# FlyCole/Dream2Real

Hardware: AMD Instinct MI355X
Metric: candidate renders scored/sec (640x360) (higher is better)
Workload: dtype bf16 + fp16 NeRF MLP operands (fp32 accumulate; the library's default: the reference's tiny-cuda-nn operand type, same MFMA rate; --opt mlp_f16=0 = bf16 operands)

## Files before the change

### dream2real_amd/_lib.py

```python
from __future__ import annotations

import ctypes as C
import os

import numpy as np

_HERE = os.path.dirname(os.path.abspath(__file__))
LIB_PATH = os.path.join(_HERE, "libd2r.so")
ABI_VERSION = 10

EXPORTS = [
    "d2r_abi_version", "d2r_ctx_create", "d2r_ctx_destroy", "d2r_ctx_set_stream", "d2r_ctx_synchronize",
    "d2r_last_error", "d2r_nerf_create", "d2r_nerf_destroy", "d2r_render", "d2r_nerf_eval_points",
    "d2r_set_background", "d2r_render_composite", "d2r_clip_create", "d2r_clip_destroy",
    "d2r_clip_score_frames", "d2r_clip_preprocess", "d2r_clip_embed_pixels", "d2r_render_score",
    "d2r_get_render_stats", "d2r_collect_render_stats", "d2r_ctx_set_option", "d2r_get_timing", "d2r_text_create",
    "d2r_text_destroy", "d2r_text_encode", "d2r_comm_get_unique_id", "d2r_comm_init", "d2r_comm_destroy",
    "d2r_allgather_scores", "d2r_phys_create", "d2r_phys_destroy", "d2r_phys_check", "d2r_nerf_load_ingp", "d2r_lens_undistort_view",
    "d2r_rectify_background_depth", "d2r_ingp_inspect", "d2r_render_score_host", "d2r_png_write", "d2r_png_write_batch",
    "d2r_png_read_batch", "d2r_png_size", "d2r_savetxt", "d2r_ingp_validate", "d2r_debug_gemm_fp8", "d2r_ctx_get_option", "d2r_png_write_batch_bg",
    "d2r_pcd_create", "d2r_pcd_destroy", "d2r_pcd_render", "d2r_pcd_render_score_host",
    "d2r_tsdf_create", "d2r_tsdf_destroy", "d2r_tsdf_integrate", "d2r_tsdf_read_voxels", "d2r_tsdf_extract", "d2r_obj_write",
    "d2r_tsdf_grid", "d2r_tsdf_touch_bits", "d2r_tsdf_solid_points",
    "d2r_sdfphys_create", "d2r_sdfphys_destroy", "d2r_sdfphys_check", "d2r_sdfphys_get_timing",
    "d2r_png_write_channels", "d2r_png_info", "d2r_png_read_grey", "d2r_png_read_rgb",
    "d2r_scene_bound_masks", "d2r_masks_prune", "d2r_masks_components", "d2r_masks_lut", "d2r_masks_get_timing",
    "d2r_pcd_build", "d2r_pcd_size", "d2r_pcd_read", "d2r_pcd_build_get_timing",
    "d2r_masks_census",
]


class D2RError(RuntimeError):
    pass


class NerfDesc(C.Structure):
    _fields_ = [("n_levels", C.c_uint32), ("n_features", C.c_uint32), ("level_scale", C.c_void_p),
                ("level_res", C.c_void_p), ("level_size", C.c_void_p), ("level_offset", C.c_void_p),
                ("n_entries", C.c_uint32), ("grid_fp16", C.c_void_p), ("dw1_fp16", C.c_void_p),
                ("dw2_fp16", C.c_void_p), ("cw1_fp16", C.c_void_p), ("cw2_fp16", C.c_void_p),
                ("cw3_fp16", C.c_void_p), ("occupancy_bits", C.c_void_p), ("aabb_scale", C.c_uint32),
                ("render_aabb", C.c_float * 6)]

# ... 308 lines not shown

def pcd_build_timing(ctx):
    ms = np.zeros(2, np.float64)
    check(load().d2r_pcd_build_get_timing(_h(ctx), ptr(ms)), _h(ctx))
    return tuple(float(x) for x in ms)


def ingp_validate(data: bytes) -> IngpInfo:
    info = IngpInfo()
    lib = load()
    lib.d2r_ingp_validate.argtypes = [C.c_char_p, C.c_size_t, C.c_void_p]
    check(lib.d2r_ingp_validate(data, len(data), C.byref(info)))
    return info


def check(rc: int, ctx=None):
    if rc != 0:
        msg = load().d2r_last_error(ctx)
        raise D2RError(f"libd2r error {rc}: {msg.decode() if msg else '?'}")


def ptr(a) -> C.c_void_p:
    if a is None:
        return C.c_void_p(0)
    assert a.flags["C_CONTIGUOUS"]
    return C.c_void_p(a.ctypes.data)


def view_c(v) -> ViewC:
    return ViewC(v.width, v.height, (C.c_float * 2)(*v.focal), (C.c_float * 2)(*v.center), v.scale,
# ... 3 lines not shown
```

### dream2real_amd/csrc/api.hip

```cpp
#include <math.h>
#include <string.h>

#include <algorithm>
#include <chrono>

#include "d2r_internal.h"
#include "pngio.h"

struct d2r_clip;
int d2r_launch_preprocess(d2r_ctx *, d2r_clip *, const uint8_t *frames_dev, uint32_t n, uint32_t w, uint32_t h,
                          int rot90, uint16_t *patches_dev, float *pixel_values_dev, const void *rects_dev = nullptr,
                          const uint16_t *bg_patches_dev = nullptr, bool touched_only = false);
bool d2r_clip_l0_supported(const d2r_ctx *, const d2r_clip *);
int d2r_clip_forward(d2r_ctx *, const d2r_clip *, const uint16_t *patches_dev, uint32_t n, const float *text_dev,
                     uint32_t C, float logit_scale, float *logits_dev, float *embeds_dev, const ClipL0Reuse *reuse = nullptr);
int d2r_clip_layer0_background(d2r_ctx *, const d2r_clip *, const uint16_t *bg_patches_dev, ClipL0Reuse *out);
int d2r_launch_patchify(d2r_ctx *, const d2r_clip *, const float *pv_dev, uint32_t n, uint16_t *patches_dev);
size_t d2r_clip_patch_bytes(const d2r_clip *, uint32_t n);
int d2r_launch_eval_points(d2r_ctx *, const d2r_nerf *, const float *xyz, const float *dirs, uint32_t n, float *out);
uint32_t d2r_clip_image_size(const d2r_clip *);
uint32_t d2r_clip_proj_dim(const d2r_clip *);
uint32_t d2r_clip_max_images(const d2r_clip *);
uint32_t d2r_clip_tokens(const d2r_clip *);

uint32_t d2r_pass_size(const d2r_ctx *ctx, const d2r_clip *clip, size_t px)
{
    uint64_t per = (uint64_t)std::max<int64_t>(1, ctx->chunk);
// ... 140 lines not shown
    {"ray_sort_log2", &d2r_ctx::ray_sort_log2, Option::RANGE, 1, 4},
    {"march_threads", &d2r_ctx::march_threads, Option::RANGE, 0, D2R_MARCH_THREADS, 0, opt_march_threads},
    {"march_threads_auto_mib", &d2r_ctx::march_threads_auto_mib, Option::RANGE, 0, 1 << 20},
    {"march_blocks", &d2r_ctx::march_blocks, Option::RANGE, 0, 65535},
    {"gemm_cfg", &d2r_ctx::gemm_cfg, Option::FREE, 0, 0, OPT_DEV},
    {"gemm_group", &d2r_ctx::gemm_group, Option::RANGE, 0, 65535, OPT_DEV},
    {"gemm_stagger", &d2r_ctx::gemm_stagger, Option::FLAG, 0, 0, OPT_DEV},
    {"gbrick_slots", &d2r_ctx::gbrick_slots, Option::RANGE, 0, 8},
    {"brick_slots_total", &d2r_ctx::brick_slots_total, Option::RANGE, 0, 8},
    {"lds_slots_max", &d2r_ctx::lds_slots_max, Option::RANGE, 0, 5},
    {"gbrick_max_mib", &d2r_ctx::gbrick_max_mib, Option::RANGE, 0, 512},
    {"mlp_f16", &d2r_ctx::mlp_f16, Option::FLAG},
    {"render_arith", &d2r_ctx::render_arith, Option::RANGE, 0, 2},
    {"bricks", &d2r_ctx::use_bricks, Option::FLAG},
    {"raygen_rect", &d2r_ctx::raygen_rect, Option::FLAG},
    {"timing", &d2r_ctx::timing, Option::RANGE, 0, 2, 0, opt_timing},
    {"march_lds_slots", &d2r_ctx::last_march_nb, Option::FREE, 0, 0, OPT_READ_ONLY},
    {"march_hbm_brick_slots", &d2r_ctx::last_march_ngb, Option::FREE, 0, 0, OPT_READ_ONLY},
    {"march_hbm_brick_bytes", &d2r_ctx::last_march_gbrick_bytes, Option::FREE, 0, 0, OPT_READ_ONLY},
    {"march_threads_used", &d2r_ctx::last_march_threads, Option::FREE, 0, 0, OPT_READ_ONLY},
};

static const Option *find_option(const char *key)
{
    for (const Option &o : g_options)
        if (!strcmp(key, o.key)) return (o.flags & OPT_DEV) && !kDevBuild ? nullptr : &o;
    return nullptr;
}

size_t d2r_ctx::timing_begin(int kind)
// ... 749 lines not shown
    ClipL0Reuse l0{};
    const bool use_l0 = reuse_bg && ctx->l0_reuse && d2r_clip_l0_supported(ctx, clip);
    if (use_l0) {
        if (ctx->bg_l0_for != (const void *)clip) {
            rc = d2r_clip_layer0_background(ctx, clip, (const uint16_t *)ctx->bg_patches.p, &ctx->bg_l0_desc);
            if (rc == D2R_OK) ctx->bg_l0_for = (const void *)clip;
            else if (rc != D2R_ERR_UNSUPPORTED) return rc;
        }
        if (ctx->bg_l0_for == (const void *)clip) {
            l0 = ctx->bg_l0_desc;
            l0.w = V.W;
            l0.h = V.H;
            l0.rects = ctx->rects.p;
        }
    }
    ctx->stats = d2r_render_stats{};
    hipStream_t main = ctx->stream, rs = two ? ctx->render_stream : main, xs = ctx->copy_stream;
    if (rs != main) {
        D2R_HIP(ctx, hipEventRecord(ctx->ev_fork, main));
        D2R_HIP(ctx, hipStreamWaitEvent(rs, ctx->ev_fork, 0));
    }
    uint32_t prev_c0 = 0, prev_nc = 0;
    int prev_b = -1;
    for (uint32_t c0 = 0, ci = 0; c0 < K; c0 += per, ci++) {
        const uint32_t nc = std::min(per, K - c0);
        const int b = (int)(ci & 1u), pb = two ? b : 0, fbuf = (to_host && nchunks > 1) ? b : 0;
        uint8_t *frames_dev = (uint8_t *)(fbuf ? ctx->frames2.p : ctx->frames.p);
        uint16_t *patches = (uint16_t *)(pb ? ctx->patches2.p : ctx->clipws[6].p);
        void *rects = reuse_bg ? (void *)((uint8_t *)ctx->rects.p + (size_t)pb * cap * 16) : nullptr;
        if (to_host && ci >= 2) ctx->pool->wait(b);
        {
            StreamSwap sw(ctx, rs);
            if (to_host && ci >= 2) D2R_HIP(ctx, hipStreamWaitEvent(rs, ctx->ev_copy[b], 0));
            if (two && ci >= 2) D2R_HIP(ctx, hipStreamWaitEvent(rs, ctx->ev_clip[pb], 0));
            if ((rc = d2r_launch_cameras_virtual(ctx, V, obj_pose_now, cam_pose, poses_dev + (size_t)c0 * 16, nc, (float *)ctx->cams.p)))
                return rc;
            if ((rc = d2r_launch_render(ctx, fg, V, (const float *)ctx->cams.p, nc, true, nullptr, nullptr, frames_dev, rects)))
                return rc;
            D2R_HIP(ctx, hipMemcpyAsync((uint8_t *)ctx->counters.p + 64 + 32 * (size_t)ci, ctx->counters.p, 32,
                                        hipMemcpyDeviceToDevice, rs));
            if (ctx->debug_fail_chunk >= 0 && (int64_t)ci == ctx->debug_fail_chunk) {
                ctx->debug_fail_chunk = -1;
                return d2r_fail(ctx, D2R_ERR_DEVICE, "injected fault in chunk " + std::to_string(ci) + " (option debug_fail_chunk)");
            }
            size_t tp = ctx->timing_begin(D2R_T_PREP);
            if ((rc = d2r_launch_preprocess(ctx, (d2r_clip *)clip, frames_dev, nc, V.W, V.H, 1, patches, nullptr, rects,
                                            reuse_bg ? (const uint16_t *)ctx->bg_patches.p : nullptr, l0.rects != nullptr)))
                return rc;
            ctx->timing_end(tp);
            if (to_host) {
                D2R_HIP(ctx, hipEventRecord(ctx->ev_march[b], rs));
                D2R_HIP(ctx, hipStreamWaitEvent(xs, ctx->ev_march[b], 0));
// ... 127 lines not shown
    ctx->stats.samples = 0;
    ctx->stats.wave_iters = 0;
    ctx->stats.l0_touched = 0;
    for (uint32_t i = 0; i < nchunks; i++) {
        if (ctx->stats.l0_tokens) ctx->stats.l0_touched += c[i * 8 + 6];
        uint64_t s, it;
        memcpy(&s, &c[i * 8 + 2], 8);
        memcpy(&it, &c[i * 8 + 4], 8);
        ctx->stats.rays_alive += c[i * 8];
        ctx->stats.samples += s;
        ctx->stats.wave_iters += it;
    }
    return D2R_OK;
}

}
```

### dream2real_amd/csrc/clip.hip

```cpp
#include "d2r_internal.h"

#include <type_traits>

#include <math.h>
#include <stdio.h>
#include <stdlib.h>

#include <algorithm>
#include <deque>
#include <mutex>

typedef __bf16 bf16x8 __attribute__((ext_vector_type(8)));
typedef float f32x16 __attribute__((ext_vector_type(16)));
typedef float f32x4 __attribute__((ext_vector_type(4)));

struct ClipWeights {
    const uint16_t *w_patch;
    const float *cls, *pos;
    const float *pre_w, *pre_b;
    struct Layer {
        const float *ln1_w, *ln1_b, *ln2_w, *ln2_b;
        const uint16_t *w_qkv, *w_o, *w_fc1, *w_fc2;
        const float *b_qkv, *b_o, *b_fc1, *b_fc2;
        const uint16_t *wf_qkv = nullptr, *wf_fc1 = nullptr;
// ... 9 lines not shown
    const int *kk_h;
    const int *bounds_v;
    const int *kk_v;
    int ks_h, ks_v;
    int need_h, need_v;
    int iw, ih;
    int rw, rh;
    int left, top;
    int max_rows;
};

struct PrepCache {
    uint32_t w, h;
    int rot90;
    ResampleTables R;
};

struct d2r_clip {
    d2r_ctx *ctx;
    d2r_clip_desc desc;
    uint32_t T, Kp, Kp_pad;
    std::vector<void *> allocs;
    ClipWeights w;
    std::vector<ClipWeights::Layer> layers;
    std::deque<PrepCache> prep;
    std::mutex prep_mu;
    struct F8Layer { const uint8_t *w_qkv, *w_o, *w_fc1, *w_fc2; float s_qkv, s_o, s_fc1, s_fc2; };
    std::vector<F8Layer> f8;
    std::mutex f8_mu;
};
// ... 2416 lines not shown
        for (int x = 0; x < xmax; x++) {
            k[x] = bicubic_filter((x + xmin - center + 0.5) * ss);
            ww += k[x];
        }
        for (int x = 0; x < ksize; x++) {
            double v = x < xmax ? (ww != 0.0 ? k[x] / ww : k[x]) : 0.0;
            kk[(size_t)xx * ksize + x] = v < 0 ? (int)(-0.5 + v * (1 << PRECISION_BITS))
                                               : (int)(0.5 + v * (1 << PRECISION_BITS));
        }
        bounds[xx * 2] = xmin;
        bounds[xx * 2 + 1] = xmax;
    }
    return ksize;
}

static int prep_tables(d2r_ctx *ctx, d2r_clip *clip, uint32_t w, uint32_t h, int rot90, const PrepCache **out)
{
    std::lock_guard<std::mutex> lock(clip->prep_mu);
    for (const PrepCache &pc : clip->prep)
        if (pc.w == w && pc.h == h && pc.rot90 == rot90) {
            *out = &pc;
            return D2R_OK;
        }
    const uint32_t S = clip->desc.image_size, P = clip->desc.patch_size;
    ResampleTables R{};
    R.iw = rot90 ? (int)h : (int)w;
    R.ih = rot90 ? (int)w : (int)h;
    int short_e = R.iw < R.ih ? R.iw : R.ih, long_e = R.iw < R.ih ? R.ih : R.iw;
    int new_long = (int)((double)S * long_e / short_e);
    R.rw = R.iw <= R.ih ? (int)S : new_long;
    R.rh = R.iw <= R.ih ? new_long : (int)S;
    R.need_h = R.rw != R.iw;
    R.need_v = R.rh != R.ih;
    R.left = (R.rw - (int)S) / 2;
    R.top = (R.rh - (int)S) / 2;
    std::vector<int> bh, kh, bv, kv;
    R.ks_h = resample_coeffs(R.iw, R.rw, bh, kh);
    R.ks_v = resample_coeffs(R.ih, R.rh, bv, kv);
    const uint32_t band = P;
    int max_rows = (int)band;
    if (R.need_v) {
        max_rows = 0;
        for (uint32_t r0 = 0; r0 < S; r0 += band) {
            uint32_t last = std::min(r0 + band, S) - 1;
            int y0 = bv[2 * (R.top + r0)], y1 = bv[2 * (R.top + last)] + bv[2 * (R.top + last) + 1];
            max_rows = std::max(max_rows, y1 - y0);
        }
    }
    R.max_rows = max_rows;
    std::vector<int> all;
    size_t o_bh = 0, o_kh = o_bh + bh.size(), o_bv = o_kh + kh.size(), o_kv = o_bv + bv.size();
    all.insert(all.end(), bh.begin(), bh.end());
    all.insert(all.end(), kh.begin(), kh.end());
    all.insert(all.end(), bv.begin(), bv.end());
    all.insert(all.end(), kv.begin(), kv.end());
    int *dev = nullptr;
    if (hipMalloc(&dev, all.size() * sizeof(int)) != hipSuccess) return d2r_fail(ctx, D2R_ERR_MEMORY, "hipMalloc failed");
    clip->allocs.push_back(dev);
    D2R_HIP(ctx, hipMemcpy(dev, all.data(), all.size() * sizeof(int), hipMemcpyHostToDevice));
    R.bounds_h = dev + o_bh;
    R.kk_h = dev + o_kh;
    R.bounds_v = dev + o_bv;
    R.kk_v = dev + o_kv;
    clip->prep.push_back(PrepCache{w, h, rot90, R});
    *out = &clip->prep.back();
    return D2R_OK;
}

int d2r_launch_preprocess(d2r_ctx *ctx, d2r_clip *clip, const uint8_t *frames_dev, uint32_t n, uint32_t w,
                          uint32_t h, int rot90, uint16_t *patches_dev, float *pixel_values_dev, const void *rects_dev,
                          const uint16_t *bg_patches_dev, bool touched_only)
{
    const uint32_t S = clip->desc.image_size, P = clip->desc.patch_size;
    const PrepCache *pc = nullptr;
    int rc = prep_tables(ctx, clip, w, h, rot90, &pc);
    if (rc) return rc;
    const ResampleTables &R = pc->R;
    const uint32_t band = P;
    size_t lds = (size_t)R.max_rows * S * 3;
    if (lds > 150 * 1024) return d2r_fail(ctx, D2R_ERR_UNSUPPORTED, "preprocess band does not fit in LDS");
// ... 823 lines not shown
```

### dream2real_amd/csrc/d2r_internal.h

```cpp
#pragma once
#include <hip/hip_runtime.h>
#include <stdint.h>

#include <functional>
#include <memory>
#include <mutex>
#include <string>
#include <utility>
#include <vector>

#include "../../include/d2r.h"
#include "d2r_shared.h"

class D2rJobPool;
struct D2rPngBase;

#define D2R_MAX_LEVELS 16
#define D2R_MAX_DEVICES 64
#define D2R_GRID 128
#define D2R_DT 0.0016914558f
#define D2R_INV_DT (1.0f / D2R_DT)
#define D2R_CONE 0.00390625f
#define D2R_T_LINEAR (D2R_DT * 256.0f)
#define D2R_N_WFRAG 24
// ... 13 lines not shown
    uint32_t hashed[2];
    uint32_t mask8;
    uint32_t off;
    uint32_t bnx[2], bnxy[2];
    int32_t bbase[2];
};

struct NerfParams {
    const uint32_t *grid;
    uint32_t grid_bytes;
    uint32_t n_levels;
    int32_t n_dense;
    SlotMeta slot[D2R_MAX_LEVELS / 2];
    uint32_t refill_min;
    uint32_t compact;
    uint32_t sort_log2;
    uint32_t n_brick_slots;
    uint32_t brick_words;
    const uint32_t *brick_tab;
    uint32_t n_gbrick_slots;
    uint32_t gbrick_bytes;
    const uint32_t *gbrick_tab;
    const uint64_t *bricks;
    uint32_t aabb_scale;
    uint32_t n_casc;
    float side, inv_side;
    const uint4 *wfrag;
    const uint4 *wfrag16;
    float bbox_lo[3], bbox_hi[3];
    float raabb_lo[3], raabb_hi[3], rn_lo[3], rn_hi[3];
// ... 82 lines not shown
    int64_t last_march_threads = 0, last_march_gbrick_bytes = 0;
    int64_t last_march_nb = 0, last_march_ngb = 0;
    int64_t refill_min = 64;
    int64_t march_compact = 1;
    int64_t ln_fold = 4;
    int64_t gemm_stagger = 0;
    int64_t gemm_group = 65535;
    int64_t gemm_nsplit = 0;
    int64_t attn_rem = 1;
    int64_t cls_last = 1;
    int64_t gemm_cfg = 0;
    int64_t mlp_f16 = 1;
    int64_t render_arith = 0;
    int64_t use_bricks = 1;
    int64_t raygen_rect = 1;
    int64_t gbrick_slots = 8;
    int64_t brick_slots_total = 7;
    int64_t lds_slots_max = 5;
    int64_t gbrick_max_mib = 512;
    int64_t timing = 0;
    std::vector<hipEvent_t> ev_pool;
    size_t ev_used = 0;
    std::vector<std::pair<int, std::pair<size_t, size_t>>> ev_pairs;
    size_t timing_begin(int kind);
    void timing_end(size_t pair);
};
enum { D2R_T_MARCH = 0, D2R_T_RAYGEN = 1, D2R_T_CLIP = 2, D2R_T_PREP = 3, D2R_T_SORT = 4,
       D2R_T_VIT_QKV = 5, D2R_T_VIT_ATTN = 6, D2R_T_VIT_OUT = 7, D2R_T_VIT_FC1 = 8, D2R_T_VIT_FC2 = 9, D2R_T_KINDS = 10 };

struct d2r_nerf {
// ... 34 lines not shown
#define D2R_HIP(ctx, expr)                                                              \
    do {                                                                                \
        hipError_t e_ = (expr);                                                         \
        if (e_ != hipSuccess)                                                           \
            return d2r_fail(ctx, D2R_ERR_DEVICE,                                        \
                            std::string(#expr) + ": " + hipGetErrorString(e_));         \
    } while (0)

int d2r_launch_cameras_direct(d2r_ctx *, const ViewParams &, const float *cams_nerf_dev, uint32_t n,
                              float *cams_out);
int d2r_launch_cameras_virtual(d2r_ctx *, const ViewParams &, const float *obj_now16,
                               const float *cam16, const float *obj_poses_dev, uint32_t n,
                               float *cams_out);
int d2r_launch_render(d2r_ctx *, const d2r_nerf *, const ViewParams &, const float *cams_dev,
                      uint32_t n, bool composite, float *rgba_dev, float *depth_dev,
                      uint8_t *frames_dev, void *rects_dev = nullptr);
int d2r_launch_bg_quantize(d2r_ctx *, uint32_t w, uint32_t h);
ViewParams d2r_view_params(const d2r_view *v);
int d2r_reserve_render(d2r_ctx *, size_t rays);
int d2r_lens_table(d2r_ctx *, ViewParams &V);
```

### dream2real_amd/csrc/nerf.hip

```cpp
#include <algorithm>
#include <cstring>

#include "d2r_internal.h"
#include <type_traits>

typedef __bf16 bf16x8 __attribute__((ext_vector_type(8)));
typedef float f32x16 __attribute__((ext_vector_type(16)));

typedef _Float16 f16x8 __attribute__((ext_vector_type(8)));
union Frag {
    bf16x8 v;
    f16x8 h;
    uint4 u;
};

template <bool F16>
__device__ __forceinline__ uint32_t pack2(float a, float b)
{
    if constexpr (F16) {
        typedef _Float16 f16x2 __attribute__((ext_vector_type(2)));
        union { f16x2 v; uint32_t u; } r;
        r.v[0] = (_Float16)a;
        r.v[1] = (_Float16)b;
        return r.u;
// ... 453 lines not shown
            uint32_t off = (uint32_t)__popcll(m & ((1ull << lane) - 1ull));
            queue[base + off] = make_uint2(ray_id, k);
        }
    }
    if (inside && !alive && rgba_out) {
        float e[4];
        empty_pixel(V, e);
        *(float4 *)(rgba_out + (size_t)ray_id * 4) = make_float4(e[0], e[1], e[2], e[3]);
        depth_out[ray_id] = 0.f;
    }
}

template <bool CONE>
__global__ __launch_bounds__(256) void k_raygen_rect(NerfParams P, ViewParams V, const float *__restrict__ cams,
                                                     uint2 *__restrict__ queue, uint32_t *__restrict__ qcount,
                                                     int4 *__restrict__ rects)
{
    if (CONE) cone_tab_to_lds();
    const uint32_t cam_i = blockIdx.x;
    const uint32_t lane = threadIdx.x & 63, wave = threadIdx.x >> 6;
    float cam[12];
#pragma unroll
    for (int j = 0; j < 12; j++) cam[j] = cams[(size_t)cam_i * 12 + j];
    int x0 = 0, y0 = 0, x1 = (int)V.W - 1, y1 = (int)V.H - 1;
    {
        bool ok = true;
#pragma unroll
        for (int a = 0; a < 3; a++)
#pragma unroll
            for (int b = a; b < 3; b++) {
                const float dot = cam[a] * cam[b] + cam[4 + a] * cam[4 + b] + cam[8 + a] * cam[8 + b];
// ... 43 lines not shown
            const float h = fmaxf(u1 - u0, v1 - v0) * (1.0f / 15.0f);
            margin += h * h * 0.125f * d2max * fmaxf(V.focal[0], V.focal[1]);
            ok = ok && detmin > 0.1f && margin < 1e6f;
            u0 = lu0; u1 = lu1; v0 = lv0; v1 = lv1;
        }
        if (ok) {
            const float pxmin = fmaf(u0, V.focal[0], V.center[0] * (float)V.W) - 0.5f, pxmax = fmaf(u1, V.focal[0], V.center[0] * (float)V.W) - 0.5f;
            const float pymin = fmaf(v0, V.focal[1], V.center[1] * (float)V.H) - 0.5f, pymax = fmaf(v1, V.focal[1], V.center[1] * (float)V.H) - 0.5f;
            const int mg = (int)ceilf(margin);
            x0 = max(x0, (int)floorf(fmaxf(pxmin, -4.f)) - mg);
            y0 = max(y0, (int)floorf(fmaxf(pymin, -4.f)) - mg);
            x1 = min(x1, (int)ceilf(fminf(pxmax, (float)V.W + 4.f)) + mg);
            y1 = min(y1, (int)ceilf(fminf(pymax, (float)V.H + 4.f)) + mg);
        }
    }
    if (x0 > x1 || y0 > y1) {
        if (rects && blockIdx.y == 0 && threadIdx.x == 0) rects[cam_i] = make_int4(1, 1, 0, 0);
        return;
    }
    const int tx0 = x0 >> 4, ty0 = y0 >> 4, ntx = (x1 >> 4) - tx0 + 1, nty = (y1 >> 4) - ty0 + 1;
    if (rects && blockIdx.y == 0 && threadIdx.x == 0)
        rects[cam_i] = make_int4(tx0 * 16, ty0 * 16, min((int)V.W, (tx0 + ntx) * 16) - 1, min((int)V.H, (ty0 + nty) * 16) - 1);
    constexpr uint32_t CAP = 2048;
    __shared__ uint2 pending[CAP];
    __shared__ uint32_t n_pending, flush_base;
    if (threadIdx.x == 0) n_pending = 0;
    __syncthreads();
    auto flush = [&]() {
        __syncthreads();
        const uint32_t np_ = n_pending;
        if (threadIdx.x == 0 && np_) flush_base = atomicAdd(qcount, np_);
        __syncthreads();
        for (uint32_t i = threadIdx.x; i < np_; i += 256) queue[flush_base + i] = pending[i];
        __syncthreads();
        if (threadIdx.x == 0) n_pending = 0;
        __syncthreads();
    };
    uint32_t since_flush = 0;
    for (int t = (int)blockIdx.y; t < ntx * nty; t += (int)gridDim.y) {
        if (since_flush + 256 > CAP) {
            flush();
            since_flush = 0;
        }
        since_flush += 256;
        const uint32_t px = (uint32_t)(tx0 + t % ntx) * 16 + (wave & 1) * 8 + (lane & 7);
        const uint32_t py = (uint32_t)(ty0 + t / ntx) * 16 + (wave >> 1) * 8 + (lane >> 3);
        bool alive = false;
        uint32_t k = 0;
        if (px < V.W && py < V.H) {
            Ray r;
            if (make_ray<CONE>(P, V, cam, px, py, r, k)) {
                float x, y, z;
                alive = next_sample<CONE>(P, r, k, x, y, z);
                if (alive) k |= sort_tag(P, x, y, z);
            }
        }
        const uint32_t ray_id = cam_i * (V.W * V.H) + py * V.W + px;
        unsigned long long m = __ballot(alive);
        if (m) {
            uint32_t cnt = (uint32_t)__popcll(m), base = 0;
            if (lane == (uint32_t)__ffsll((long long)m) - 1) base = atomicAdd(&n_pending, cnt);
            base = __shfl(base, __ffsll((long long)m) - 1);
            if (alive) {
                uint32_t off = (uint32_t)__popcll(m & ((1ull << lane) - 1ull));
// ... 583 lines not shown
    if (CONE) cone_tab_to_lds();
    __syncthreads();
    const uint32_t lane = threadIdx.x & 63;
    const uint32_t n_q = *qcount;
    const uint32_t WH = V.W * V.H;
    __amdgpu_buffer_rsrc_t rs = __builtin_amdgcn_make_buffer_rsrc((void *)P.grid, 0, P.grid_bytes, 0x00020000);
    __amdgpu_buffer_rsrc_t rsb = __builtin_amdgcn_make_buffer_rsrc((void *)P.gbrick_tab, 0, P.gbrick_bytes, 0x00020000);

    bool alive = false, exhausted = false;
    uint32_t res_lo = 0, res_hi = 0;
    Ray ray = {};
    uint32_t k = 0, ray_id = 0;
    float px = 0.f, py = 0.f, pz = 0.f;
    float C0 = 0.f, C1 = 0.f, C2 = 0.f, A = 0.f, Z = 0.f;
    float zslope = 0.f, zbase = 0.f;
    uint32_t nsamp = 0, niter = 0;
    uint4 shfA = make_uint4(0, 0, 0, 0), shfB = shfA;

#if D2R_MARCH_PROF
    long long prof_t0 = clock64(), prof_refill = 0;
    uint32_t prof_n = 0, prof_le32 = 0, prof_le16 = 0, prof_half = 0, prof_alive = 0;
#endif
    for (;;) {
        bool sh_dirty = false;
        if (P.compact) {
            const unsigned long long am = __ballot(alive);
            const uint32_t na = (uint32_t)__popcll(am);
            if (na != 0u && na <= 32u && (am >> 32) != 0ull) {
                const unsigned long long below = (1ull << lane) - 1ull;
                const uint32_t dest = alive ? (uint32_t)__popcll(am & below) : na + (uint32_t)__popcll(~am & below);
                const int d4 = (int)(dest << 2);
                auto mv = [&](float &v) { v = __int_as_float(__builtin_amdgcn_ds_permute(d4, __float_as_int(v))); };
                auto mvu = [&](uint32_t &v) { v = (uint32_t)__builtin_amdgcn_ds_permute(d4, (int)v); };
                mv(ray.ox); mv(ray.oy); mv(ray.oz); mv(ray.dx); mv(ray.dy); mv(ray.dz); mv(ray.t0); mvu(ray.k_hi);
                if (CONE) { mvu(ray.k1); mv(ray.t1); }
                mvu(k); mvu(ray_id); mv(px); mv(py); mv(pz);
                mv(C0); mv(C1); mv(C2); mv(A); mv(Z); mv(zslope); mv(zbase);
                alive = lane < na;
                sh_dirty = true;
            }
        }
        unsigned long long freem = __ballot(!alive);
        if ((!exhausted || res_lo < res_hi) && freem != 0ull && (__popcll(freem) >= (int)P.refill_min || freem == ~0ull)) {
#if D2R_MARCH_PROF
            const long long prof_a = clock64();
#endif
            const uint32_t nfree = (uint32_t)__popcll(freem);
            if (res_lo == res_hi) {
                uint32_t base = 0;
                if (lane == 0) base = atomicAdd(qhead, (uint32_t)D2R_MARCH_RESERVE);
                base = __builtin_amdgcn_readfirstlane(base);
                res_lo = min(base, n_q);
// ... 14 lines not shown
                    float cam[12];
#pragma unroll
                    for (int j = 0; j < 12; j++) cam[j] = cams[(size_t)cam_i * 12 + j];
                    uint32_t klo;
                    make_ray<CONE>(P, V, cam, pix % V.W, pix / V.W, ray, klo);
                    float t = lattice_t<CONE>(ray, k);
                    px = fmaf(t, ray.dx, ray.ox);
                    py = fmaf(t, ray.dy, ray.oy);
                    pz = fmaf(t, ray.dz, ray.oz);
                    const float wdx = CONE ? ray.dx * P.side : ray.dx, wdy = CONE ? ray.dy * P.side : ray.dy, wdz = CONE ? ray.dz * P.side : ray.dz;
                    const float wox = CONE ? fmaf(ray.ox - 0.5f, P.side, 0.5f) : ray.ox, woy = CONE ? fmaf(ray.oy - 0.5f, P.side, 0.5f) : ray.oy;
                    const float woz = CONE ? fmaf(ray.oz - 0.5f, P.side, 0.5f) : ray.oz;
                    zslope = (wdx * cam[2] + wdy * cam[6] + wdz * cam[10]) * V.inv_scale;
                    zbase = ((wox - cam[3]) * cam[2] + (woy - cam[7]) * cam[6] + (woz - cam[11]) * cam[10]) * V.inv_scale;
                    C0 = C1 = C2 = A = Z = 0.f;
                    alive = true;
                }
            }
            sh_dirty = true;
#if D2R_MARCH_PROF
            asm volatile("s_waitcnt vmcnt(0) lgkmcnt(0)" ::: "memory");
            prof_refill += clock64() - prof_a;
            prof_n++;
#endif
        }
        if (!__any(alive)) break;
        if (sh_dirty) {
            if (CONE) sh_fragments<F16>(lane, ray.dx * P.side, ray.dy * P.side, ray.dz * P.side, shfA, shfB);
            else sh_fragments<F16>(lane, ray.dx, ray.dy, ray.dz, shfA, shfB);
        }
// ... 17 lines not shown
        eval_wave<NB, NGB, ND, F16, ARITH>(P, rs, rsb, sw, lds_bricks, lane, alive, px, py, pz, shfA, shfB, sigma, cr, cg, cb);

        if (alive) {
            nsamp++;
            float T = 1.0f - A;
            const float tk = lattice_t<CONE>(ray, k);
            float alpha = 1.0f - expf(-sigma * lattice_dt<CONE>(tk));
            float wgt = alpha * T;
            float zz = fmaf(tk, zslope, zbase);
            C0 = fmaf(wgt, cr, C0);
            C1 = fmaf(wgt, cg, C1);
            C2 = fmaf(wgt, cb, C2);
            Z = fmaf(wgt, zz, Z);
            A += wgt;
            bool done = false;
            if (A > 1.0f - V.min_transmittance) {
                float ia = 1.0f / A;
                C0 *= ia; C1 *= ia; C2 *= ia; Z *= ia;
                A = 1.0f;
                done = true;
            } else {
                k++;
#if (D2R_MARCH_VAR & 2)
                done = !next_sample<CONE>(P, ray, k, px, py, pz, &occ_next);
#else
                done = !next_sample<CONE>(P, ray, k, px, py, pz);
#endif
            }
            if (done) {
                alive = false;
                float o0 = fmaf((1.0f - A) * V.background[3], V.background[0], srgb_to_linear(C0));
// ... 138 lines not shown
}

int d2r_reserve_render(d2r_ctx *ctx, size_t rays)
{
    int rc;
    if ((rc = d2r_reserve(ctx, ctx->queue, rays * sizeof(uint2)))) return rc;
    if (ctx->ray_sort) {
        const size_t max_chunks = (rays + D2R_SORT_CHUNK - 1) / D2R_SORT_CHUNK;
        if ((rc = d2r_reserve(ctx, ctx->queue2, rays * sizeof(uint2)))) return rc;
        if ((rc = d2r_reserve(ctx, ctx->sort_counts, (max_chunks + 2) * D2R_SORT_BINS * 4))) return rc;
    }
    return D2R_OK;
}

int d2r_launch_render(d2r_ctx *ctx, const d2r_nerf *m, const ViewParams &V, const float *cams_dev, uint32_t n,
                      bool composite, float *rgba_dev, float *depth_dev, uint8_t *frames_dev, void *rects_dev)
{
    const size_t rays = (size_t)n * V.W * V.H;
    if (rays >= (1ull << 32)) return d2r_fail(ctx, D2R_ERR_INVALID, "too many rays in one pass");
    if (V.lens_mode == D2R_LENS_OPENCV && !V.lens_tab)
        return d2r_fail(ctx, D2R_ERR_INVALID, "d2r_launch_render: a view with a lens arrived without its table (d2r_lens_table)");
    int rc;
    if ((rc = d2r_reserve_render(ctx, rays))) return rc;
    if ((rc = d2r_reserve(ctx, ctx->counters, 64))) return rc;
    uint32_t *cnt = (uint32_t *)ctx->counters.p;
    D2R_HIP(ctx, hipMemsetAsync(cnt, 0, 32, ctx->stream));
    if (composite) {
        if (ctx->bg_w != V.W || ctx->bg_h != V.H || !ctx->bg_u8.p)
            return d2r_fail(ctx, D2R_ERR_INVALID, "d2r_set_background must be called for this view first");
        const uint32_t n_bytes = V.W * V.H * 3;
        if (n_bytes % 16 == 0) {
            const uint32_t n_vec = n_bytes / 16;
            hipLaunchKernelGGL(k_frames_init, dim3((n_vec + 255) / 256, n < 64 ? n : 64), dim3(256), 0, ctx->stream,
                               (const uint4 *)ctx->bg_u8.p, (uint4 *)frames_dev, n_vec, n);
        } else {
            hipLaunchKernelGGL(k_frames_init_bytes, dim3((n_bytes + 255) / 256, n < 64 ? n : 64), dim3(256), 0,
                               ctx->stream, (const uint8_t *)ctx->bg_u8.p, frames_dev, n_bytes, n);
        }
    }
    const uint32_t tiles = ((V.W + 15) / 16) * ((V.H + 15) / 16);
    const uint32_t sort_log2 = ctx->ray_sort ? (uint32_t)ctx->ray_sort_log2 : 0u;
    NerfParams PR = m->P;
    PR.sort_log2 = sort_log2;
    size_t tr = ctx->timing_begin(D2R_T_RAYGEN);
    const bool cone = m->P.aabb_scale >= 2;
    if (composite && ctx->raygen_rect) {
        if (cone) hipLaunchKernelGGL(k_raygen_rect<true>, dim3(n, 4), dim3(256), 0, ctx->stream, PR, V, cams_dev, (uint2 *)ctx->queue.p, cnt, (int4 *)rects_dev);
        else hipLaunchKernelGGL(k_raygen_rect<false>, dim3(n, 4), dim3(256), 0, ctx->stream, PR, V, cams_dev, (uint2 *)ctx->queue.p, cnt, (int4 *)rects_dev);
    } else {
        if (cone)
            hipLaunchKernelGGL(k_raygen<true>, dim3(tiles, n), dim3(256), 0, ctx->stream, PR, V, cams_dev, (uint2 *)ctx->queue.p,
                               cnt, composite ? nullptr : rgba_dev, composite ? nullptr : depth_dev);
        else
            hipLaunchKernelGGL(k_raygen<false>, dim3(tiles, n), dim3(256), 0, ctx->stream, PR, V, cams_dev, (uint2 *)ctx->queue.p,
                               cnt, composite ? nullptr : rgba_dev, composite ? nullptr : depth_dev);
    }
    ctx->timing_end(tr);
    const uint2 *q = (const uint2 *)ctx->queue.p;
    if (sort_log2) {
        size_t ts = ctx->timing_begin(D2R_T_SORT);
        const size_t max_chunks = (rays + D2R_SORT_CHUNK - 1) / D2R_SORT_CHUNK;
        uint32_t *counts = (uint32_t *)ctx->sort_counts.p, *bin_total = counts + max_chunks * D2R_SORT_BINS, *bin_base = bin_total + D2R_SORT_BINS;
        const int sb = (int)std::min<size_t>(max_chunks, 4096);
// ... 20 lines not shown
            case 4: ngb = ngb >= 3 ? 3 : ngb >= 2 ? 2 : 0; break;
            case 3: case 2: case 1:
                if (ngb >= 7 - nb) ngb = 7 - nb;
                else if (ngb >= 6 - nb) ngb = 6 - nb;
                else none = true;
                break;
            default: ngb = ngb >= 7 ? 7 : ngb >= 6 ? 6 : 0; break;
        }
        if (none) nb = ngb = 0;
    }
    const int arith = (int)ctx->render_arith;
    if (arith) nb = ngb = 0;
    NerfParams PP = m->P;
    PP.refill_min = (uint32_t)ctx->refill_min;
    PP.compact = (uint32_t)ctx->march_compact;
    const size_t lds = (size_t)D2R_N_WFRAG * 64 * 16 + (nb ? (size_t)m->P.brick_words * 4 : 0);
    uint32_t threads = D2R_MARCH_THREADS;
    if (ctx->march_threads > 0) threads = std::min<uint32_t>((uint32_t)ctx->march_threads, D2R_MARCH_THREADS);
    else if (!sort_log2 && ngb && m->P.gbrick_bytes > (size_t)ctx->march_threads_auto_mib << 20) threads = std::min<uint32_t>(512u, D2R_MARCH_THREADS);
#define D2R_MARCH_C(COMP, NB, NGB, ND, CONE)                            \
    do {                                                                \
        if (ctx->mlp_f16) D2R_MARCH_F(COMP, NB, NGB, ND, CONE, true, 0);   \
        else D2R_MARCH_F(COMP, NB, NGB, ND, CONE, false, 0);               \
    } while (0)
#define D2R_MARCH_F(COMP, NB, NGB, ND, CONE, F16, ARITH)                                                              \
    do {                                                                                                          \
        static PerDeviceOnce attr;                                                                                \
        attr.run(ctx->device, [] {                                                                                \
            (void)hipFuncSetAttribute((const void *)k_march<COMP, NB, NGB, ND, CONE, F16, ARITH>, hipFuncAttributeMaxDynamicSharedMemorySize, 160 * 1024 - (CONE ? 512 : 0));  \
        });                                                                                                       \
// ... 74 lines not shown
```

### dream2real_amd/engine.py

```python
from __future__ import annotations

import ctypes as C
import dataclasses
import os

import numpy as np

from . import _lib
from .clip_model import pack_text_weights, pack_vision_weights
from .scene import LENS_OPENCV, LENS_PERSPECTIVE, NerfModel, View

Shade = "Shade"
Depth = "Depth"


class Context:

    def __init__(self, device: int = 0):
        self.lib = _lib.load()
        h = C.c_void_p()
        _lib.check(self.lib.d2r_ctx_create(C.c_int(device), C.byref(h)))
        self.h = h
        self.device = device

# ... 20 lines not shown
    def set_option(self, key: str, value: int):
        self.check(self.lib.d2r_ctx_set_option(self.h, key.encode(), C.c_int64(value)))

    def get_option(self, key: str) -> int:
        v = C.c_int64(0)
        self.check(self.lib.d2r_ctx_get_option(self.h, key.encode(), C.byref(v)))
        return int(v.value)

    def render_stats(self, collect_K: int | None = None) -> dict:
        if collect_K is not None:
            self.check(self.lib.d2r_collect_render_stats(self.h, C.c_uint32(collect_K)))
        s = _lib.RenderStats()
        self.check(self.lib.d2r_get_render_stats(self.h, C.byref(s)))
        return {"rays_total": s.rays_total, "rays_alive": s.rays_alive, "samples": s.samples,
                "wave_iters": s.wave_iters, "l0_tokens": s.l0_tokens, "l0_touched": s.l0_touched}

    def timing(self) -> dict:
        t = _lib.Timing()
        self.check(self.lib.d2r_get_timing(self.h, C.byref(t)))
        return {k: getattr(t, k) for k, _ in t._fields_}

    def comm_unique_id(self) -> bytes:
        buf = C.create_string_buffer(_lib.COMM_ID_BYTES)
        _lib.check(self.lib.d2r_comm_get_unique_id(buf))
        return buf.raw

    def comm_init(self, id_blob: bytes | None, rank: int, world: int):
        if id_blob is not None:
            assert len(id_blob) == _lib.COMM_ID_BYTES
        self.check(self.lib.d2r_comm_init(self.h, id_blob, C.c_int(rank), C.c_int(world)))
# ... 301 lines not shown
```

### include/d2r.h

```cpp
#ifndef D2R_H
#define D2R_H

#include <stddef.h>
#include <stdint.h>

#ifdef __cplusplus
extern "C" {
#endif

#define D2R_API __attribute__((visibility("default")))
#define D2R_ABI_VERSION 10

typedef enum {
    D2R_OK = 0,
    D2R_ERR_INVALID = -1,
    D2R_ERR_DEVICE = -2,
    D2R_ERR_MEMORY = -3,
    D2R_ERR_UNSUPPORTED = -4
} d2r_status;

typedef struct d2r_ctx d2r_ctx;
typedef struct d2r_nerf d2r_nerf;
typedef struct d2r_clip d2r_clip;

// ... 96 lines not shown
} d2r_clip_desc;

D2R_API int d2r_clip_create(d2r_ctx *ctx, const d2r_clip_desc *desc, const float *weights,
                            size_t n_floats, d2r_clip **out);
D2R_API void d2r_clip_destroy(d2r_clip *clip);

D2R_API int d2r_clip_score_frames(d2r_ctx *ctx, const d2r_clip *clip, const uint8_t *frames,
                                  uint32_t n, uint32_t w, uint32_t h, int rot90,
                                  const float *text_embeds, uint32_t C, float logit_scale,
                                  float *logits_out, float *embeds_out);

D2R_API int d2r_clip_preprocess(d2r_ctx *ctx, const d2r_clip *clip, const uint8_t *frames,
                                uint32_t n, uint32_t w, uint32_t h, int rot90,
                                float *pixel_values_out);

D2R_API int d2r_clip_embed_pixels(d2r_ctx *ctx, const d2r_clip *clip, const float *pixel_values,
                                  uint32_t n, float *embeds_out);

D2R_API int d2r_debug_gemm_fp8(d2r_ctx *ctx, const float *A, const float *W, const float *bias, uint32_t M, uint32_t N,
                               uint32_t K, int kind, float *out, uint8_t *a_q8, uint8_t *a_scales, float *w_scale_out,
                               uint8_t *out_q8, uint8_t *out_scales);


typedef struct {
    uint32_t vocab_size;
    uint32_t context_length;
    uint32_t hidden_size;
    uint32_t num_layers;
    uint32_t num_heads;
    uint32_t mlp_size;
// ... 36 lines not shown
D2R_API int d2r_png_read_batch(const char *dir, const uint32_t *indices, uint32_t first_index, uint32_t n, uint32_t w,
                               uint32_t h, uint8_t *frames_out, int threads);
D2R_API int d2r_png_size(const char *path, uint32_t *w, uint32_t *h);
D2R_API int d2r_savetxt(const char *path, const double *data, uint64_t rows, uint64_t cols, int threads);

typedef struct {
    uint64_t rays_total;
    uint64_t rays_alive;
    uint64_t samples;
    uint64_t wave_iters;
    uint64_t l0_tokens;
    uint64_t l0_touched;
} d2r_render_stats;
D2R_API int d2r_get_render_stats(d2r_ctx *ctx, d2r_render_stats *out);
D2R_API int d2r_collect_render_stats(d2r_ctx *ctx, uint32_t K);

typedef struct {
    double march_ms;   uint64_t march_launches;
    double raygen_ms;  uint64_t raygen_launches;
    double prep_ms;    uint64_t prep_launches;
    double clip_ms;    uint64_t clip_launches;
    double sort_ms;    uint64_t sort_launches;
    double vit_qkv_ms;  uint64_t vit_qkv_launches;
    double vit_attn_ms; uint64_t vit_attn_launches;
    double vit_out_ms;  uint64_t vit_out_launches;
    double vit_fc1_ms;  uint64_t vit_fc1_launches;
    double vit_fc2_ms;  uint64_t vit_fc2_launches;
} d2r_timing;
D2R_API int d2r_get_timing(d2r_ctx *ctx, d2r_timing *out);

// ... 117 lines not shown
```

Before: 28150.

## Crop raygen to CLIP read window and exit rays occluded by background

```diff
diff --git a/dream2real_amd/_lib.py b/dream2real_amd/_lib.py
--- a/dream2real_amd/_lib.py
+++ b/dream2real_amd/_lib.py
@@ -27,6 +27,7 @@
     "d2r_scene_bound_masks", "d2r_masks_prune", "d2r_masks_components", "d2r_masks_lut", "d2r_masks_get_timing",
     "d2r_pcd_build", "d2r_pcd_size", "d2r_pcd_read", "d2r_pcd_build_get_timing",
     "d2r_masks_census",
+    "d2r_clip_read_window", "d2r_debug_read_frames", "d2r_debug_read_rays",
 ]
 
 
@@ -365,6 +366,12 @@
     return info
 
 
+def clip_read_window(width: int, height: int, image_size: int, rot90: bool = True) -> tuple:
+    win = (C.c_int32 * 4)()
+    check(load().d2r_clip_read_window(C.c_uint32(width), C.c_uint32(height), C.c_int(int(rot90)), C.c_uint32(image_size), win))
+    return tuple(int(v) for v in win)
+
+
 def check(rc: int, ctx=None):
     if rc != 0:
         msg = load().d2r_last_error(ctx)
diff --git a/dream2real_amd/csrc/api.hip b/dream2real_amd/csrc/api.hip
--- a/dream2real_amd/csrc/api.hip
+++ b/dream2real_amd/csrc/api.hip
@@ -11,6 +11,7 @@
 int d2r_launch_preprocess(d2r_ctx *, d2r_clip *, const uint8_t *frames_dev, uint32_t n, uint32_t w, uint32_t h,
                           int rot90, uint16_t *patches_dev, float *pixel_values_dev, const void *rects_dev = nullptr,
                           const uint16_t *bg_patches_dev = nullptr, bool touched_only = false);
+int d2r_clip_window(d2r_ctx *, const d2r_clip *, uint32_t w, uint32_t h, int rot90, int win[4]);
 bool d2r_clip_l0_supported(const d2r_ctx *, const d2r_clip *);
 int d2r_clip_forward(d2r_ctx *, const d2r_clip *, const uint16_t *patches_dev, uint32_t n, const float *text_dev,
                      uint32_t C, float logit_scale, float *logits_dev, float *embeds_dev, const ClipL0Reuse *reuse = nullptr);
@@ -181,6 +182,7 @@
     {"render_arith", &d2r_ctx::render_arith, Option::RANGE, 0, 2},
     {"bricks", &d2r_ctx::use_bricks, Option::FLAG},
     {"raygen_rect", &d2r_ctx::raygen_rect, Option::FLAG},
+    {"crop_rays", &d2r_ctx::crop_rays, Option::RANGE, 0, 2},
     {"timing", &d2r_ctx::timing, Option::RANGE, 0, 2, 0, opt_timing},
     {"march_lds_slots", &d2r_ctx::last_march_nb, Option::FREE, 0, 0, OPT_READ_ONLY},
     {"march_hbm_brick_slots", &d2r_ctx::last_march_ngb, Option::FREE, 0, 0, OPT_READ_ONLY},
@@ -960,6 +962,10 @@
             l0.rects = ctx->rects.p;
         }
     }
+    int window[4];
+    const bool crop = !to_host && ctx->crop_rays && ctx->raygen_rect;
+    if (crop && (rc = d2r_clip_window(ctx, clip, V.W, V.H, 1, window))) return rc;
+    const bool occluded_exit = crop && ctx->crop_rays >= 2;
     ctx->stats = d2r_render_stats{};
     hipStream_t main = ctx->stream, rs = two ? ctx->render_stream : main, xs = ctx->copy_stream;
     if (rs != main) {
@@ -981,7 +987,8 @@
             if (two && ci >= 2) D2R_HIP(ctx, hipStreamWaitEvent(rs, ctx->ev_clip[pb], 0));
             if ((rc = d2r_launch_cameras_virtual(ctx, V, obj_pose_now, cam_pose, poses_dev + (size_t)c0 * 16, nc, (float *)ctx->cams.p)))
                 return rc;
-            if ((rc = d2r_launch_render(ctx, fg, V, (const float *)ctx->cams.p, nc, true, nullptr, nullptr, frames_dev, rects)))
+            if ((rc = d2r_launch_render(ctx, fg, V, (const float *)ctx->cams.p, nc, true, nullptr, nullptr, frames_dev, rects,
+                                        crop ? window : nullptr, occluded_exit)))
                 return rc;
             D2R_HIP(ctx, hipMemcpyAsync((uint8_t *)ctx->counters.p + 64 + 32 * (size_t)ci, ctx->counters.p, 32,
                                         hipMemcpyDeviceToDevice, rs));
@@ -1139,4 +1146,33 @@
     return D2R_OK;
 }
 
-}
+int d2r_debug_read_frames(d2r_ctx *ctx, uint32_t n, uint32_t w, uint32_t h, uint8_t *frames_out)
+{
+    if (!ctx || !frames_out) return d2r_fail(ctx, D2R_ERR_INVALID, "null argument");
+    const size_t bytes = (size_t)n * w * h * 3;
+    if (!ctx->frames.p || bytes == 0 || bytes > ctx->frames.cap)
+        return d2r_fail(ctx, D2R_ERR_INVALID, "d2r_debug_read_frames: the context holds no such frames");
+    D2R_HIP(ctx, hipStreamSynchronize(ctx->stream));
+    D2R_HIP(ctx, hipMemcpy(frames_out, ctx->frames.p, bytes, hipMemcpyDeviceToHost));
+    return D2R_OK;
+}
+
+int d2r_debug_read_rays(d2r_ctx *ctx, uint32_t cap, uint32_t *ray_ids_out, uint32_t *n_out)
+{
+    if (!ctx || !n_out || (cap && !ray_ids_out)) return d2r_fail(ctx, D2R_ERR_INVALID, "null argument");
+    if (!ctx->queue.p || !ctx->counters.p) return d2r_fail(ctx, D2R_ERR_INVALID, "d2r_debug_read_rays: the context has rendered nothing");
+    D2R_HIP(ctx, hipStreamSynchronize(ctx->stream));
+    uint32_t n = 0;
+    D2R_HIP(ctx, hipMemcpy(&n, ctx->counters.p, 4, hipMemcpyDeviceToHost));
+    if ((size_t)n * sizeof(uint2) > ctx->queue.cap) return d2r_fail(ctx, D2R_ERR_INVALID, "d2r_debug_read_rays: stale ray count");
+    *n_out = n;
+    const uint32_t m = std::min(n, cap);
+    if (m) {
+        std::vector<uint32_t> q((size_t)m * 2);
+        D2R_HIP(ctx, hipMemcpy(q.data(), ctx->queue.p, q.size() * 4, hipMemcpyDeviceToHost));
+        for (uint32_t i = 0; i < m; i++) ray_ids_out[i] = q[2 * (size_t)i];
+    }
+    return D2R_OK;
+}
+
+}
diff --git a/dream2real_amd/csrc/clip.hip b/dream2real_amd/csrc/clip.hip
--- a/dream2real_amd/csrc/clip.hip
+++ b/dream2real_amd/csrc/clip.hip
@@ -47,6 +47,7 @@
     uint32_t w, h;
     int rot90;
     ResampleTables R;
+    int win[4];
 };
 
 struct d2r_clip {
@@ -2493,16 +2494,10 @@
     return ksize;
 }
 
-static int prep_tables(d2r_ctx *ctx, d2r_clip *clip, uint32_t w, uint32_t h, int rot90, const PrepCache **out)
-{
-    std::lock_guard<std::mutex> lock(clip->prep_mu);
-    for (const PrepCache &pc : clip->prep)
-        if (pc.w == w && pc.h == h && pc.rot90 == rot90) {
-            *out = &pc;
-            return D2R_OK;
-        }
-    const uint32_t S = clip->desc.image_size, P = clip->desc.patch_size;
-    ResampleTables R{};
+static void prep_geometry(uint32_t w, uint32_t h, int rot90, uint32_t S, ResampleTables &R, std::vector<int> &bh, std::vector<int> &kh,
+                          std::vector<int> &bv, std::vector<int> &kv)
+{
+    R = ResampleTables{};
     R.iw = rot90 ? (int)h : (int)w;
     R.ih = rot90 ? (int)w : (int)h;
     int short_e = R.iw < R.ih ? R.iw : R.ih, long_e = R.iw < R.ih ? R.ih : R.iw;
@@ -2513,9 +2508,58 @@
     R.need_v = R.rh != R.ih;
     R.left = (R.rw - (int)S) / 2;
     R.top = (R.rh - (int)S) / 2;
-    std::vector<int> bh, kh, bv, kv;
     R.ks_h = resample_coeffs(R.iw, R.rw, bh, kh);
     R.ks_v = resample_coeffs(R.ih, R.rh, bv, kv);
+}
+
+static void prep_window(const ResampleTables &R, const std::vector<int> &bh, const std::vector<int> &bv, uint32_t w, int rot90,
+                        uint32_t S, int win[4])
+{
+    int c0 = R.left, c1 = R.left + (int)S - 1, r0 = R.top, r1 = R.top + (int)S - 1;
+    if (R.need_h) {
+        c0 = INT_MAX; c1 = INT_MIN;
+        for (int ox = R.left; ox < R.left + (int)S; ox++) {
+            c0 = std::min(c0, bh[2 * ox]);
+            c1 = std::max(c1, bh[2 * ox] + bh[2 * ox + 1] - 1);
+        }
+    }
+    if (R.need_v) {
+        r0 = INT_MAX; r1 = INT_MIN;
+        for (int oy = R.top; oy < R.top + (int)S; oy++) {
+            r0 = std::min(r0, bv[2 * oy]);
+            r1 = std::max(r1, bv[2 * oy] + bv[2 * oy + 1] - 1);
+        }
+    }
+    if (rot90) { win[0] = (int)w - 1 - r1; win[1] = c0; win[2] = (int)w - 1 - r0; win[3] = c1; }
+    else { win[0] = c0; win[1] = r0; win[2] = c1; win[3] = r1; }
+}
+
+extern "C" int d2r_clip_read_window(uint32_t w, uint32_t h, int rot90, uint32_t image_size, int32_t *window_out)
+{
+    if (!w || !h || !image_size || !window_out || w > 16384 || h > 16384 || image_size > 4096) return D2R_ERR_INVALID;
+    ResampleTables R;
+    std::vector<int> bh, kh, bv, kv;
+    prep_geometry(w, h, rot90 != 0, image_size, R, bh, kh, bv, kv);
+    int win[4];
+    prep_window(R, bh, bv, w, rot90 != 0, image_size, win);
+    for (int i = 0; i < 4; i++) window_out[i] = win[i];
+    return D2R_OK;
+}
+
+static int prep_tables(d2r_ctx *ctx, d2r_clip *clip, uint32_t w, uint32_t h, int rot90, const PrepCache **out)
+{
+    std::lock_guard<std::mutex> lock(clip->prep_mu);
+    for (const PrepCache &pc : clip->prep)
+        if (pc.w == w && pc.h == h && pc.rot90 == rot90) {
+            *out = &pc;
+            return D2R_OK;
+        }
+    const uint32_t S = clip->desc.image_size, P = clip->desc.patch_size;
+    ResampleTables R;
+    std::vector<int> bh, kh, bv, kv;
+    prep_geometry(w, h, rot90, S, R, bh, kh, bv, kv);
+    PrepCache entry{w, h, rot90, R, {0, 0, 0, 0}};
+    prep_window(R, bh, bv, w, rot90, S, entry.win);
     const uint32_t band = P;
     int max_rows = (int)band;
     if (R.need_v) {
@@ -2541,8 +2585,18 @@
     R.kk_h = dev + o_kh;
     R.bounds_v = dev + o_bv;
     R.kk_v = dev + o_kv;
-    clip->prep.push_back(PrepCache{w, h, rot90, R});
+    entry.R = R;
+    clip->prep.push_back(entry);
     *out = &clip->prep.back();
+    return D2R_OK;
+}
+
+int d2r_clip_window(d2r_ctx *ctx, const d2r_clip *clip, uint32_t w, uint32_t h, int rot90, int win[4])
+{
+    const PrepCache *pc = nullptr;
+    int rc = prep_tables(ctx, (d2r_clip *)clip, w, h, rot90, &pc);
+    if (rc) return rc;
+    for (int i = 0; i < 4; i++) win[i] = pc->win[i];
     return D2R_OK;
 }
 
diff --git a/dream2real_amd/csrc/d2r_internal.h b/dream2real_amd/csrc/d2r_internal.h
--- a/dream2real_amd/csrc/d2r_internal.h
+++ b/dream2real_amd/csrc/d2r_internal.h
@@ -51,6 +51,7 @@
     SlotMeta slot[D2R_MAX_LEVELS / 2];
     uint32_t refill_min;
     uint32_t compact;
+    uint32_t occluded_exit;
     uint32_t sort_log2;
     uint32_t n_brick_slots;
     uint32_t brick_words;
@@ -163,6 +164,7 @@
     int64_t render_arith = 0;
     int64_t use_bricks = 1;
     int64_t raygen_rect = 1;
+    int64_t crop_rays = 1;
     int64_t gbrick_slots = 8;
     int64_t brick_slots_total = 7;
     int64_t lds_slots_max = 5;
@@ -227,7 +229,8 @@
                                float *cams_out);
 int d2r_launch_render(d2r_ctx *, const d2r_nerf *, const ViewParams &, const float *cams_dev,
                       uint32_t n, bool composite, float *rgba_dev, float *depth_dev,
-                      uint8_t *frames_dev, void *rects_dev = nullptr);
+                      uint8_t *frames_dev, void *rects_dev = nullptr,
+                      const int *window = nullptr, bool occluded_exit = false);
 int d2r_launch_bg_quantize(d2r_ctx *, uint32_t w, uint32_t h);
 ViewParams d2r_view_params(const d2r_view *v);
 int d2r_reserve_render(d2r_ctx *, size_t rays);
diff --git a/dream2real_amd/csrc/nerf.hip b/dream2real_amd/csrc/nerf.hip
--- a/dream2real_amd/csrc/nerf.hip
+++ b/dream2real_amd/csrc/nerf.hip
@@ -491,7 +491,7 @@
 template <bool CONE>
 __global__ __launch_bounds__(256) void k_raygen_rect(NerfParams P, ViewParams V, const float *__restrict__ cams,
                                                      uint2 *__restrict__ queue, uint32_t *__restrict__ qcount,
-                                                     int4 *__restrict__ rects)
+                                                     int4 *__restrict__ rects, int4 win)
 {
     if (CONE) cone_tab_to_lds();
     const uint32_t cam_i = blockIdx.x;
@@ -565,13 +565,16 @@
             y1 = min(y1, (int)ceilf(fminf(pymax, (float)V.H + 4.f)) + mg);
         }
     }
+    x0 = max(x0, win.x); y0 = max(y0, win.y);
+    x1 = min(x1, win.z); y1 = min(y1, win.w);
     if (x0 > x1 || y0 > y1) {
         if (rects && blockIdx.y == 0 && threadIdx.x == 0) rects[cam_i] = make_int4(1, 1, 0, 0);
         return;
     }
     const int tx0 = x0 >> 4, ty0 = y0 >> 4, ntx = (x1 >> 4) - tx0 + 1, nty = (y1 >> 4) - ty0 + 1;
     if (rects && blockIdx.y == 0 && threadIdx.x == 0)
-        rects[cam_i] = make_int4(tx0 * 16, ty0 * 16, min((int)V.W, (tx0 + ntx) * 16) - 1, min((int)V.H, (ty0 + nty) * 16) - 1);
+        rects[cam_i] = make_int4(max(tx0 * 16, win.x), max(ty0 * 16, win.y), min(min((int)V.W, (tx0 + ntx) * 16) - 1, win.z),
+                                 min(min((int)V.H, (ty0 + nty) * 16) - 1, win.w));
     constexpr uint32_t CAP = 2048;
     __shared__ uint2 pending[CAP];
     __shared__ uint32_t n_pending, flush_base;
@@ -598,7 +601,7 @@
         const uint32_t py = (uint32_t)(ty0 + t / ntx) * 16 + (wave >> 1) * 8 + (lane >> 3);
         bool alive = false;
         uint32_t k = 0;
-        if (px < V.W && py < V.H) {
+        if ((int)px >= win.x && (int)px <= win.z && (int)py >= win.y && (int)py <= win.w) {
             Ray r;
             if (make_ray<CONE>(P, V, cam, px, py, r, k)) {
                 float x, y, z;
@@ -1212,6 +1215,7 @@
     float px = 0.f, py = 0.f, pz = 0.f;
     float C0 = 0.f, C1 = 0.f, C2 = 0.f, A = 0.f, Z = 0.f;
     float zslope = 0.f, zbase = 0.f;
+    float zlim = INFINITY;
     uint32_t nsamp = 0, niter = 0;
     uint4 shfA = make_uint4(0, 0, 0, 0), shfB = shfA;
 
@@ -1234,6 +1238,7 @@
                 if (CONE) { mvu(ray.k1); mv(ray.t1); }
                 mvu(k); mvu(ray_id); mv(px); mv(py); mv(pz);
                 mv(C0); mv(C1); mv(C2); mv(A); mv(Z); mv(zslope); mv(zbase);
+                if (COMPOSITE) mv(zlim);
                 alive = lane < na;
                 sh_dirty = true;
             }
@@ -1278,6 +1283,10 @@
                     zslope = (wdx * cam[2] + wdy * cam[6] + wdz * cam[10]) * V.inv_scale;
                     zbase = ((wox - cam[3]) * cam[2] + (woy - cam[7]) * cam[6] + (woz - cam[11]) * cam[10]) * V.inv_scale;
                     C0 = C1 = C2 = A = Z = 0.f;
+                    if (COMPOSITE && P.occluded_exit) {
+                        const float bd = bg_depth[pix];
+                        zlim = bd < 0.05f ? 100.f : bd;
+                    }
                     alive = true;
                 }
             }
@@ -1325,7 +1334,10 @@
             Z = fmaf(wgt, zz, Z);
             A += wgt;
             bool done = false;
-            if (A > 1.0f - V.min_transmittance) {
+            const bool occluded = COMPOSITE && Z >= 0.05f && Z >= zlim;
+            if (occluded) {
+                alive = false;
+            } else if (A > 1.0f - V.min_transmittance) {
                 float ia = 1.0f / A;
                 C0 *= ia; C1 *= ia; C2 *= ia; Z *= ia;
                 A = 1.0f;
@@ -1494,7 +1506,8 @@
 }
 
 int d2r_launch_render(d2r_ctx *ctx, const d2r_nerf *m, const ViewParams &V, const float *cams_dev, uint32_t n,
-                      bool composite, float *rgba_dev, float *depth_dev, uint8_t *frames_dev, void *rects_dev)
+                      bool composite, float *rgba_dev, float *depth_dev, uint8_t *frames_dev, void *rects_dev,
+                      const int *window, bool occluded_exit)
 {
     const size_t rays = (size_t)n * V.W * V.H;
     if (rays >= (1ull << 32)) return d2r_fail(ctx, D2R_ERR_INVALID, "too many rays in one pass");
@@ -1525,8 +1538,10 @@
     size_t tr = ctx->timing_begin(D2R_T_RAYGEN);
     const bool cone = m->P.aabb_scale >= 2;
     if (composite && ctx->raygen_rect) {
-        if (cone) hipLaunchKernelGGL(k_raygen_rect<true>, dim3(n, 4), dim3(256), 0, ctx->stream, PR, V, cams_dev, (uint2 *)ctx->queue.p, cnt, (int4 *)rects_dev);
-        else hipLaunchKernelGGL(k_raygen_rect<false>, dim3(n, 4), dim3(256), 0, ctx->stream, PR, V, cams_dev, (uint2 *)ctx->queue.p, cnt, (int4 *)rects_dev);
+        int4 win = make_int4(0, 0, (int)V.W - 1, (int)V.H - 1);
+        if (window) win = make_int4(std::max(window[0], 0), std::max(window[1], 0), std::min(window[2], win.z), std::min(window[3], win.w));
+        if (cone) hipLaunchKernelGGL(k_raygen_rect<true>, dim3(n, 4), dim3(256), 0, ctx->stream, PR, V, cams_dev, (uint2 *)ctx->queue.p, cnt, (int4 *)rects_dev, win);
+        else hipLaunchKernelGGL(k_raygen_rect<false>, dim3(n, 4), dim3(256), 0, ctx->stream, PR, V, cams_dev, (uint2 *)ctx->queue.p, cnt, (int4 *)rects_dev, win);
     } else {
         if (cone)
             hipLaunchKernelGGL(k_raygen<true>, dim3(tiles, n), dim3(256), 0, ctx->stream, PR, V, cams_dev, (uint2 *)ctx->queue.p,
@@ -1577,6 +1592,7 @@
     NerfParams PP = m->P;
     PP.refill_min = (uint32_t)ctx->refill_min;
     PP.compact = (uint32_t)ctx->march_compact;
+    PP.occluded_exit = composite && occluded_exit ? 1u : 0u;
     const size_t lds = (size_t)D2R_N_WFRAG * 64 * 16 + (nb ? (size_t)m->P.brick_words * 4 : 0);
     uint32_t threads = D2R_MARCH_THREADS;
     if (ctx->march_threads > 0) threads = std::min<uint32_t>((uint32_t)ctx->march_threads, D2R_MARCH_THREADS);
diff --git a/dream2real_amd/engine.py b/dream2real_amd/engine.py
--- a/dream2real_amd/engine.py
+++ b/dream2real_amd/engine.py
@@ -58,6 +58,18 @@
         self.check(self.lib.d2r_get_render_stats(self.h, C.byref(s)))
         return {"rays_total": s.rays_total, "rays_alive": s.rays_alive, "samples": s.samples,
                 "wave_iters": s.wave_iters, "l0_tokens": s.l0_tokens, "l0_touched": s.l0_touched}
+
+    def read_frames(self, n: int, width: int, height: int) -> np.ndarray:
+        frames = np.empty((n, height, width, 3), np.uint8)
+        self.check(self.lib.d2r_debug_read_frames(self.h, C.c_uint32(n), C.c_uint32(width), C.c_uint32(height), _lib.ptr(frames)))
+        return frames
+
+    def read_rays(self) -> np.ndarray:
+        n = C.c_uint32(0)
+        self.check(self.lib.d2r_debug_read_rays(self.h, C.c_uint32(0), None, C.byref(n)))
+        ids = np.empty(n.value, np.uint32)
+        self.check(self.lib.d2r_debug_read_rays(self.h, C.c_uint32(n.value), _lib.ptr(ids), C.byref(n)))
+        return ids
 
     def timing(self) -> dict:
         t = _lib.Timing()
diff --git a/include/d2r.h b/include/d2r.h
--- a/include/d2r.h
+++ b/include/d2r.h
@@ -134,6 +134,8 @@
                                 uint32_t n, uint32_t w, uint32_t h, int rot90,
                                 float *pixel_values_out);
 
+D2R_API int d2r_clip_read_window(uint32_t w, uint32_t h, int rot90, uint32_t image_size, int32_t *window_out);
+
 D2R_API int d2r_clip_embed_pixels(d2r_ctx *ctx, const d2r_clip *clip, const float *pixel_values,
                                   uint32_t n, float *embeds_out);
 
@@ -200,6 +202,8 @@
 } d2r_render_stats;
 D2R_API int d2r_get_render_stats(d2r_ctx *ctx, d2r_render_stats *out);
 D2R_API int d2r_collect_render_stats(d2r_ctx *ctx, uint32_t K);
+D2R_API int d2r_debug_read_frames(d2r_ctx *ctx, uint32_t n, uint32_t w, uint32_t h, uint8_t *frames_out);
+D2R_API int d2r_debug_read_rays(d2r_ctx *ctx, uint32_t cap, uint32_t *ray_ids_out, uint32_t *n_out);
 
 typedef struct {
     double march_ms;   uint64_t march_launches;
```

Result: no change. 28320, median of 6 (+0.6%).
